# ameli/gaussian-process-param-estimation

Hardware: AMD Instinct MI355X
Metric: log-likelihood evals/sec (N=16384 dense Matern-3/2) (higher is better)
Workload: dtype f64

## Files before the change

### gaussian-process-param-estimation_amd/csrc/gpmi_api.hip

```cpp

#include <hip/hip_runtime.h>

#include <algorithm>
#include <cmath>
#include <cstdarg>
#include <cstdio>
#include <cstdlib>
#include <cstring>
#include <array>
#include <map>
#include <vector>

#include "gpmi_internal.h"
#include "gpmi_host.h"
#include "gpmi_band.h"
#include "../../include/gpmi.h"

using namespace gpmi;

namespace {

thread_local char g_err[512] = "";

int set_err(int code, const char* fmt, ...) {
  va_list ap;
  va_start(ap, fmt);
  vsnprintf(g_err, sizeof(g_err), fmt, ap);
  va_end(ap);
  return code;
}

constexpr int TS = GPMI_TS;
constexpr int RLD = GPMI_RHS_LD;
constexpr int OUT_LD = 1 + RLD * RLD;

}

struct gpmi_op {
  int device = 0;
  int64_t n = 0, n_pad = 0;
  int nt = 0;
  int max_batch = 1;
  int outer = 16;
  hipStream_t stream = nullptr;
  hipStream_t stream3 = nullptr;
  int groups = 0;
  hipEvent_t ev_g = nullptr;
  hipEvent_t ev_fork = nullptr, ev_join = nullptr;
  bool dry = false;
  std::vector<std::pair<int, int>> shapes;
  double* K = nullptr;
  double* A = nullptr;
  double* R = nullptr;
  double* X = nullptr;
  double* U = nullptr;
  double* Linv = nullptr;
  double* logdiag = nullptr;
  double* gram = nullptr;
  double* out = nullptr;
  double* etas = nullptr;
  double* rhs_src = nullptr;
  double* scratch = nullptr;
  double* scratch2 = nullptr;
  double* tracebuf = nullptr;
  double* W = nullptr;
  double* tpart = nullptr;
  double* Td = nullptr;
  int* info = nullptr;
  uint32_t* order = nullptr;
  int order_nt = -1, order_outer = -1, group = 8;
  std::map<std::pair<int, int>, int64_t> order_off;
  int nrhs = 0;
  bool has_K = false;
  bool cache_valid = false;
  double cached_eta = 0.0;
  uint64_t factor_gen = 0;
  uint64_t tinv_gen = ~0ull;
  int tinv_have = 0;
  double tinv[2] = {0.0, 0.0};
  bool timing = false;
  std::vector<hipEvent_t> ev;
  hipEvent_t ev_begin = nullptr, ev_end = nullptr;
  double last_syrk_ms = 0.0, last_syrk_flops = 0.0, last_total_ms = 0.0;
  int last_syrk_launches = 0;
  std::vector<std::pair<int, double>> syrk_log;
  std::vector<std::array<int, 3>> syrk_shape;
  double last_syrk_busy_ms = 0.0;

  BatchPtrs ptrs() const {
    BatchPtrs p;
    p.A = A;
    p.sA = n_pad * n_pad;
    p.R = R;
    p.sR = n_pad * RLD;
    p.U = U;
    p.sU = (int64_t)TS * RLD;
    p.Linv = Linv;
    p.sL = (int64_t)nt * TS * TS;
    p.logdiag = logdiag;
    p.sLD = nt;
    p.gram = gram;
    p.sG = (int64_t)nt * 256;
    p.info = info;
    return p;
  }
};

namespace {

void grouped_order(int w, int t, int G, std::vector<uint32_t>* out) {
  for (int r0 = 0; r0 < t; r0 += G) {
    const int r1 = std::min(t, r0 + G);
    const int jmax = std::min(r1 - 1, w - 1);
    for (int j = 0; j <= jmax; ++j)
      for (int i = std::max(r0, j); i < r1; ++i) out->push_back(((uint32_t)i << 16) | j);
  }
}

int launch_syrk(gpmi_op* op, hipStream_t st, int b0, int nb, int tc0, int w, int t, int p0,
                int kdim, bool from_k = false) {
  const int tri = w * (w + 1) / 2;
  const int tiles = tri + (t - w) * w;
  if (tiles <= 0 || nb <= 0) return 0;
  if (op->dry) {
    op->shapes.push_back({w, t});
    return 0;
  }
  int evi = -1;
  if (op->timing) {
    evi = (int)op->syrk_log.size() * 2;
    if ((int)op->ev.size() < evi + 2) {
      for (int k = 0; k < 64; ++k) {
        hipEvent_t e;
        HIP_TRY(hipEventCreateWithFlags(&e, timing_event_flags()));
        op->ev.push_back(e);
      }
    }
    HIP_TRY(hipEventRecord(op->ev[evi], st));
  }
  const uint32_t* order = nullptr;
  if (op->order && w > 1) {
    auto it = op->order_off.find({w, t});
    if (it != op->order_off.end()) order = op->order + it->second;
  }
  hipLaunchKernelGGL(syrk_kernel, dim3(tiles, nb), dim3(256), 0, st,
                     op->A + (int64_t)b0 * op->n_pad * op->n_pad, (int64_t)op->n_pad,
                     op->n_pad * op->n_pad, tc0, w, t, p0, kdim, order,
                     from_k ? op->K : nullptr, op->etas + b0, (int64_t)op->n);
  LAUNCH_CHECK("syrk_kernel");
  if (op->timing) {
    HIP_TRY(hipEventRecord(op->ev[evi + 1], st));
    const double offd = (double)(tiles - std::min(tiles, w)) * TS * TS;
    const double diag = (double)std::min(tiles, w) * TS * (TS + 1) / 2.0;
    const double fl = 2.0 * (offd + diag) * kdim * nb;
    op->syrk_log.push_back({evi, fl});
    op->syrk_shape.push_back({w, t, kdim});
  }
  return 0;
}

int factor_panel(gpmi_op* op, const BatchPtrs& P, int b0, int nb, hipStream_t st, int c0,
                 int W) {
  const int nt = op->nt;
  if (W == 1) {
    if (op->dry) return 0;
    hipLaunchKernelGGL(diag_block_kernel, dim3(nb), dim3(256), 0, st, P, (int64_t)op->n_pad,
                       c0, nt);
    LAUNCH_CHECK("diag_block_kernel");
    if (c0 + 1 < nt) {
      hipLaunchKernelGGL(panel_kernel, dim3(nt - c0 - 1, nb), dim3(256), 0, st, P,
                         (int64_t)op->n_pad, c0);
      LAUNCH_CHECK("panel_kernel");
    }
    return 0;
  }
  const int h = W / 2;
  int rc = factor_panel(op, P, b0, nb, st, c0, h);
  if (rc) return rc;
  rc = launch_syrk(op, st, b0, nb, c0 + h, W - h, nt - c0 - h, c0 * TS, h * TS);
  if (rc) return rc;
  return factor_panel(op, P, b0, nb, st, c0 + h, W - h);
}


int schedule(gpmi_op* op, const BatchPtrs& P, int b0, int nb, hipStream_t main = nullptr) {
  const int nt = op->nt, O = op->outer;
  hipStream_t A = main ? main : op->stream;
  for (int c0 = 0; c0 < nt; c0 += O) {
    const int W = std::min(O, nt - c0);
    int rc = factor_panel(op, P, b0, nb, A, c0, W);
    if (rc) return rc;
    const int c1 = c0 + W;
    if (c1 >= nt) break;
    rc = launch_syrk(op, A, b0, nb, c1, nt - c1, nt - c1, c0 * TS, W * TS, c0 == 0);
    if (rc) return rc;
  }
  return 0;
}

int ensure_order(gpmi_op* op) {
  if (op->group <= 0) return 0;
  if (op->order && op->order_nt == op->nt && op->order_outer == op->outer &&
      true)
    return 0;
  if (op->order) HIP_TRY(hipFree(op->order));
  op->order = nullptr;
  op->order_off.clear();
  op->dry = true;
  op->shapes.clear();
  BatchPtrs P = op->ptrs();
  int rc = schedule(op, P, 0, 1);
  op->dry = false;
  if (rc) return rc;
  std::vector<uint32_t> h;
  for (auto& wt : op->shapes) {
    if (wt.first < 2 || op->order_off.count(wt)) continue;
    op->order_off[wt] = (int64_t)h.size();
    grouped_order(wt.first, wt.second, op->group, &h);
  }
  if (h.empty()) h.push_back(0);
  HIP_TRY(hipMalloc(&op->order, sizeof(uint32_t) * h.size()));
  HIP_TRY(hipMemcpy(op->order, h.data(), sizeof(uint32_t) * h.size(), hipMemcpyHostToDevice));
  op->order_nt = op->nt;
  op->order_outer = op->outer;
  return 0;
}

BatchPtrs shifted(const BatchPtrs& P, int b0) {
  BatchPtrs q = P;
  q.A += b0 * P.sA;
  q.R += b0 * P.sR;
  q.U += b0 * P.sU;
  q.Linv += b0 * P.sL;
  q.logdiag += b0 * P.sLD;
  q.gram += b0 * P.sG;
  q.info += b0;
  return q;
}

int run_factor(gpmi_op* op, const double* etas_host, int nb, const double* rhs_dev) {
  if (!op->has_K) return set_err(-1000, "operator has no matrix (load or assemble first)");
  if (nb < 1 || nb > op->max_batch)
    return set_err(-1001, "batch %d outside [1, %d]", nb, op->max_batch);
  DeviceGuard g(op->device);
  hipStream_t s = op->stream;
  const int nt = op->nt;
  const int64_t lda = op->n_pad;
  BatchPtrs P = op->ptrs();
  {
    int rc = ensure_order(op);
    if (rc) return rc;
  }
  op->syrk_log.clear();
  op->syrk_shape.clear();
  op->cache_valid = false;
  ++op->factor_gen;
  if (op->timing) {
    if (!op->ev_begin) {
      HIP_TRY(hipEventCreateWithFlags(&op->ev_begin, timing_event_flags()));
      HIP_TRY(hipEventCreateWithFlags(&op->ev_end, timing_event_flags()));
    }
    HIP_TRY(hipEventRecord(op->ev_begin, s));
  }
  HIP_TRY(hipMemcpyAsync(op->etas, etas_host, sizeof(double) * nb, hipMemcpyHostToDevice, s));
  const int wc = std::min(op->outer, nt);
  hipLaunchKernelGGL(shift_copy_kernel, dim3(wc * (wc + 1) / 2 + (nt - wc) * wc), dim3(256), 0,
                     s, op->K, lda, op->A, lda, P.sA, op->etas, nb, op->n, wc);
  LAUNCH_CHECK("shift_copy_kernel");
  for (int b = 0; b < nb; ++b)
    HIP_TRY(hipMemcpyAsync(op->R + b * P.sR, rhs_dev, sizeof(double) * P.sR,
                           hipMemcpyDeviceToDevice, s));
  HIP_TRY(hipMemsetAsync(op->info, 0, sizeof(int) * nb, s));
  int rc = 0;
  const int groups = op->groups ? op->groups : (nb <= 32 ? 2 : 1);
  if (groups == 2 && nb >= 2) {
    const int h = nb / 2;
    if (!op->stream3) {
      HIP_TRY(hipStreamCreateWithFlags(&op->stream3, hipStreamNonBlocking));
      HIP_TRY(hipEventCreateWithFlags(&op->ev_g, sync_event_flags()));
    }
    HIP_TRY(hipEventRecord(op->ev_fork, s));
    HIP_TRY(hipStreamWaitEvent(op->stream3, op->ev_fork, 0));
    if ((rc = schedule(op, P, 0, h, s))) return rc;
    if ((rc = schedule(op, shifted(P, h), h, nb - h, op->stream3))) return rc;
    HIP_TRY(hipEventRecord(op->ev_g, op->stream3));
    HIP_TRY(hipStreamWaitEvent(s, op->ev_g, 0));
  } else {
    rc = schedule(op, P, 0, nb);
  }
  if (rc) return rc;
  hipLaunchKernelGGL(finalize_kernel, dim3(nb), dim3(256), 0, s, P, nt, op->out, OUT_LD);
  LAUNCH_CHECK("finalize_kernel");
  if (op->timing) HIP_TRY(hipEventRecord(op->ev_end, s));
  return 0;
}

int collect_timing(gpmi_op* op) {
  if (!op->timing) return 0;
  HIP_TRY(hipEventSynchronize(op->ev_end));
  double tot = 0.0, fl = 0.0;
  std::vector<std::pair<double, double>> iv;
  for (auto& pr : op->syrk_log) {
    float ms = 0.f, t0 = 0.f, t1 = 0.f;
    HIP_TRY(hipEventElapsedTime(&ms, op->ev[pr.first], op->ev[pr.first + 1]));
    HIP_TRY(hipEventElapsedTime(&t0, op->ev_begin, op->ev[pr.first]));
    HIP_TRY(hipEventElapsedTime(&t1, op->ev_begin, op->ev[pr.first + 1]));
    iv.push_back({t0, t1});
    tot += ms;
    fl += pr.second;
  }
  if (std::getenv("GPMI_SYRK_TRACE")) {
    std::map<std::pair<int, int>, std::array<double, 3>> cls;
    for (size_t i = 0; i < op->syrk_log.size(); ++i) {
      const auto& sh = op->syrk_shape[i];
      float ms = 0.f;
      HIP_TRY(hipEventElapsedTime(&ms, op->ev[op->syrk_log[i].first],
                                  op->ev[op->syrk_log[i].first + 1]));
      auto& c = cls[{sh[0] == sh[1] ? 1 : 0, sh[2]}];
      c[0] += 1;
      c[1] += ms;
      c[2] += op->syrk_log[i].second;
    }
    for (auto& kv : cls)
      fprintf(stderr, "[gpmi syrk] %s kdim=%4d launches=%3.0f ms=%8.3f TF/s=%6.2f\n",
              kv.first.first ? "bulk" : "band", kv.first.second, kv.second[0], kv.second[1],
              kv.second[2] / (kv.second[1] * 1e-3) / 1e12);
  }
  std::sort(iv.begin(), iv.end());
  double busy = 0.0, cs = -1.0, ce = -1.0;
  for (auto& x : iv) {
    if (x.first > ce) {
      if (ce > cs) busy += ce - cs;
      cs = x.first;
      ce = x.second;
    } else if (x.second > ce) {
      ce = x.second;
    }
  }
  if (ce > cs) busy += ce - cs;
  float all = 0.f;
  HIP_TRY(hipEventElapsedTime(&all, op->ev_begin, op->ev_end));
  op->last_syrk_ms = tot;
  op->last_syrk_busy_ms = busy;
  op->last_syrk_flops = fl;
  op->last_syrk_launches = (int)op->syrk_log.size();
  op->last_total_ms = all;
  return 0;
}

int upload_rhs(gpmi_op* op, double* dst, const double* rhs, int64_t ld, int nrhs, int col0) {
  std::vector<double> h((size_t)op->n_pad * RLD, 0.0);
  for (int64_t i = 0; i < op->n; ++i)
    for (int c = 0; c < nrhs; ++c) h[(size_t)i * RLD + c] = rhs[i * ld + col0 + c];
  HIP_TRY(hipMemcpyAsync(dst, h.data(), sizeof(double) * h.size(),
                         hipMemcpyHostToDevice, op->stream));
  HIP_TRY(hipStreamSynchronize(op->stream));
  return 0;
}

int ensure_factor(gpmi_op* op, double eta, const double* rhs_dev, bool* fresh) {
  *fresh = false;
  if (op->cache_valid && op->cached_eta == eta) return 0;
  int rc = run_factor(op, &eta, 1, rhs_dev);
  if (rc) return rc;
  op->cache_valid = true;
  op->cached_eta = eta;
  *fresh = true;
  return 0;
}

}

namespace gpmi {
int matern_params_host(double nu, MaternParams* P);
int set_error(int code, const char* msg) { return set_err(code, "%s", msg); }
int op_view(const gpmi_op* op, OpView* v) {
  if (!op) return set_err(-1006, "null handle");
  v->device = op->device;
  v->n = op->n;
  v->n_pad = op->n_pad;
  v->K = op->K;
  v->has_K = op->has_K;
  return 0;
}
}

namespace {
__global__ void pad_identity_kernel(double* K, int64_t ldk, int64_t n) {
  const int64_t i = n + threadIdx.x;
  if (i < ldk) K[i * ldk + i] = 1.0;
}
}

extern "C" {

int gpmi_version(void) { return 100; }

int gpmi_last_error(char* buf, size_t len) {
  if (!buf || !len) return 0;
  strncpy(buf, g_err, len - 1);
  buf[len - 1] = 0;
  return 0;
}

int gpmi_device_count(int* count) {
  HIP_TRY(hipGetDeviceCount(count));
  return 0;
}

// ... 21 lines not shown
}

int gpmi_matern_values(int device, const double* x, int64_t m, double nu, double* out) {
  if (m <= 0) return 0;
  MaternParams P;
  int rc = matern_params(nu, &P);
  if (rc) return rc;
  DeviceGuard g(device);
  double *dx = nullptr, *dv = nullptr;
  HIP_TRY(hipMalloc(&dx, sizeof(double) * m));
  HIP_TRY(hipMalloc(&dv, sizeof(double) * m));
  HIP_TRY(hipMemcpy(dx, x, sizeof(double) * m, hipMemcpyHostToDevice));
  hipLaunchKernelGGL(matern_eval_kernel, dim3((unsigned)((m + 255) / 256)), dim3(256), 0, 0, dx,
                     m, P, dv);
  LAUNCH_CHECK("matern_eval_kernel");
  HIP_TRY(hipMemcpy(out, dv, sizeof(double) * m, hipMemcpyDeviceToHost));
  HIP_TRY(hipFree(dx));
  HIP_TRY(hipFree(dv));
  return 0;
}

static int assemble(int device, hipStream_t s, const double* points, int64_t n, int d,
                    const double* scale, double nu, double* Kdev, int64_t ldk,
                    int64_t n_pad) {
  if (d < 1 || d > GPMI_MAX_DIM)
    return set_err(-1003, "dimension %d outside [1, %d]", d, GPMI_MAX_DIM);
  MaternParams P;
  int rc = matern_params(nu, &P);
  if (rc) return rc;
  DeviceGuard g(device);
  double *dp = nullptr, *ds = nullptr;
  HIP_TRY(hipMalloc(&dp, sizeof(double) * std::max<int64_t>(1, n * d)));
  HIP_TRY(hipMalloc(&ds, sizeof(double) * d));
  HIP_TRY(hipMemcpyAsync(dp, points, sizeof(double) * n * d, hipMemcpyHostToDevice, s));
  HIP_TRY(hipMemcpyAsync(ds, scale, sizeof(double) * d, hipMemcpyHostToDevice, s));
  const int64_t T = (n_pad + 63) / 64;
  hipEvent_t e0 = nullptr, e1 = nullptr;
  HIP_TRY(hipEventCreate(&e0));
  HIP_TRY(hipEventCreate(&e1));
  HIP_TRY(hipEventRecord(e0, s));
  launch_matern_dense(dim3((unsigned)(T * (T + 1) / 2)), s, dp, n, d, ds, P, Kdev, ldk, n_pad);
  LAUNCH_CHECK("matern_dense_kernel");
  HIP_TRY(hipEventRecord(e1, s));
  HIP_TRY(hipStreamSynchronize(s));
  float ms = 0.f;
  HIP_TRY(hipEventElapsedTime(&ms, e0, e1));
  g_assembly_ms = ms;
  HIP_TRY(hipEventDestroy(e0));
  HIP_TRY(hipEventDestroy(e1));
  HIP_TRY(hipFree(dp));
  HIP_TRY(hipFree(ds));
  return 0;
}

int gpmi_matern_dense(int device, const double* points, int64_t n, int d,
                      const double* scale, double nu, double* K_out, int64_t ldk) {
  if (n <= 0) return 0;
  DeviceGuard g(device);
  double* dK = nullptr;
  HIP_TRY(hipMalloc(&dK, sizeof(double) * n * n));
  int rc = assemble(device, nullptr, points, n, d, scale, nu, dK, n, n);
  if (rc) {
    (void)hipFree(dK);
    return rc;
  }
  HIP_TRY(hipMemcpy2D(K_out, sizeof(double) * ldk, dK, sizeof(double) * n, sizeof(double) * n,
                      n, hipMemcpyDeviceToHost));
  HIP_TRY(hipFree(dK));
  return 0;
}

int gpmi_op_create(int device, int64_t n, int max_batch, gpmi_op** out) {
  if (!out) return set_err(-1004, "null output handle");
  if (n <= 0) return set_err(-1005, "matrix size must be positive");
  if (max_batch < 1) max_batch = 1;
  DeviceGuard g(device);
  gpmi_op* op = new gpmi_op();
  op->device = device;
  op->n = n;
  op->n_pad = (n + TS - 1) / TS * TS;
  op->nt = (int)(op->n_pad / TS);
  op->max_batch = max_batch;
  if (const char* g = std::getenv("GPMI_GROUPS")) op->groups = std::atoi(g);
  const int64_t np = op->n_pad;
  auto fail = [&](hipError_t e, const char* what) {
    gpmi_op_destroy(op);
    return set_err(-(int)e, "allocation of %s failed: %s", what, hipGetErrorString(e));
  };
  hipError_t e;
  if ((e = hipStreamCreateWithFlags(&op->stream, hipStreamNonBlocking)) != hipSuccess)
    return fail(e, "stream");
  if ((e = hipEventCreateWithFlags(&op->ev_fork, sync_event_flags())) != hipSuccess)
    return fail(e, "event");
  if ((e = hipEventCreateWithFlags(&op->ev_join, sync_event_flags())) != hipSuccess)
    return fail(e, "event");
#define ALLOC(ptr, count)                                                           \
  if ((e = hipMalloc(&op->ptr, sizeof(*op->ptr) * (size_t)(count))) != hipSuccess)  \
    return fail(e, #ptr);
  ALLOC(K, np * np);
  ALLOC(A, (size_t)max_batch * np * np);
  ALLOC(R, (size_t)max_batch * np * RLD);
  ALLOC(X, (size_t)max_batch * np * RLD);
  ALLOC(U, (size_t)max_batch * TS * RLD);
  ALLOC(Linv, (size_t)max_batch * op->nt * TS * TS);
  ALLOC(logdiag, (size_t)max_batch * op->nt);
  ALLOC(gram, (size_t)max_batch * op->nt * 256);
  ALLOC(out, (size_t)max_batch * OUT_LD);
  ALLOC(etas, max_batch);
  ALLOC(rhs_src, np * RLD);
  ALLOC(scratch, np * RLD);
  ALLOC(scratch2, np * RLD);
  ALLOC(tracebuf, np * 2);
  ALLOC(info, max_batch);
#undef ALLOC
  if ((e = hipMemsetAsync(op->rhs_src, 0, sizeof(double) * np * RLD, op->stream)) != hipSuccess)
    return fail(e, "rhs memset");
  if ((e = hipStreamSynchronize(op->stream)) != hipSuccess) return fail(e, "sync");
  *out = op;
  return 0;
}

int gpmi_op_destroy(gpmi_op* op) {
  if (!op) return 0;
  DeviceGuard g(op->device);
  if (op->stream) (void)hipStreamSynchronize(op->stream);
  if (op->stream3) (void)hipStreamSynchronize(op->stream3);
  double* bufs[] = {op->K, op->A, op->R, op->X, op->U, op->Linv, op->logdiag, op->gram,
                    op->out, op->etas, op->rhs_src, op->scratch, op->scratch2, op->tracebuf,
                    op->W, op->tpart, op->Td};
  for (double* p : bufs)
    if (p) (void)hipFree(p);
  if (op->info) (void)hipFree(op->info);
  if (op->order) (void)hipFree(op->order);
  for (auto e : op->ev) (void)hipEventDestroy(e);
  if (op->ev_begin) (void)hipEventDestroy(op->ev_begin);
  if (op->ev_end) (void)hipEventDestroy(op->ev_end);
  if (op->ev_fork) (void)hipEventDestroy(op->ev_fork);
  if (op->ev_join) (void)hipEventDestroy(op->ev_join);
  if (op->stream3) (void)hipStreamDestroy(op->stream3);
  if (op->ev_g) (void)hipEventDestroy(op->ev_g);
  if (op->stream) (void)hipStreamDestroy(op->stream);
  delete op;
  return 0;
}

int gpmi_op_size(const gpmi_op* op, int64_t* n, int64_t* n_pad) {
  if (!op) return set_err(-1006, "null handle");
  if (n) *n = op->n;
  if (n_pad) *n_pad = op->n_pad;
  return 0;
}

int gpmi_op_load_matrix(gpmi_op* op, const double* K_host, int64_t ldk) {
  if (!op) return set_err(-1006, "null handle");
  DeviceGuard g(op->device);
  const int64_t np = op->n_pad, n = op->n;
  std::vector<double> pad_rows;
  HIP_TRY(hipMemsetAsync(op->K, 0, sizeof(double) * np * np, op->stream));
  HIP_TRY(hipMemcpy2DAsync(op->K, sizeof(double) * np, K_host, sizeof(double) * ldk,
                           sizeof(double) * n, n, hipMemcpyHostToDevice, op->stream));
  if (np > n) {
    std::vector<double> one(1, 1.0);
    for (int64_t i = n; i < np; ++i)
      HIP_TRY(hipMemcpyAsync(op->K + i * np + i, one.data(), sizeof(double),
                             hipMemcpyHostToDevice, op->stream));
  }
  HIP_TRY(hipStreamSynchronize(op->stream));
  op->has_K = true;
  op->cache_valid = false;
  return 0;
}

int gpmi_op_load_sparse(gpmi_op* op, const gpmi_sp* sp) {
  if (!op || !sp) return set_err(-1006, "null handle");
  int64_t n_sp = 0;
  if (int rc = gpmi_sp_info(sp, &n_sp, nullptr)) return rc;
  if (n_sp != op->n) return set_err(-1005, "sparse operator has n = %lld, dense has %lld",
                                    (long long)n_sp, (long long)op->n);
  DeviceGuard g(op->device);
  const int64_t np = op->n_pad;
  HIP_TRY(hipMemsetAsync(op->K, 0, sizeof(double) * np * np, op->stream));
  if (int rc = gpmi::sp_scatter_dense(sp, op->device, op->K, np, op->stream)) return rc;
  if (np > op->n) {
    hipLaunchKernelGGL(pad_identity_kernel, dim3(1), dim3(128), 0, op->stream, op->K, np, op->n);
    HIP_TRY(hipGetLastError());
  }
  HIP_TRY(hipStreamSynchronize(op->stream));
  op->has_K = true;
  op->cache_valid = false;
  return 0;
}

int gpmi_op_assemble_matern(gpmi_op* op, const double* points, int d, const double* scale,
                            double nu) {
  if (!op) return set_err(-1006, "null handle");
  int rc = assemble(op->device, op->stream, points, op->n, d, scale, nu, op->K, op->n_pad,
                    op->n_pad);
  if (rc) return rc;
  op->has_K = true;
  op->cache_valid = false;
  return 0;
}

int gpmi_op_get_matrix(gpmi_op* op, double* K_out, int64_t ldk) {
  if (!op) return set_err(-1006, "null handle");
  DeviceGuard g(op->device);
  HIP_TRY(hipMemcpy2DAsync(K_out, sizeof(double) * ldk, op->K, sizeof(double) * op->n_pad,
                           sizeof(double) * op->n, op->n, hipMemcpyDeviceToHost, op->stream));
  HIP_TRY(hipStreamSynchronize(op->stream));
  return 0;
}

int gpmi_op_set_rhs(gpmi_op* op, const double* rhs, int64_t ld, int nrhs) {
  if (!op) return set_err(-1006, "null handle");
  if (nrhs < 0 || nrhs > RLD) return set_err(-1007, "nrhs %d outside [0, %d]", nrhs, RLD);
  DeviceGuard g(op->device);
  int rc = upload_rhs(op, op->rhs_src, rhs, ld, nrhs, 0);
// ... 268 lines not shown
```

### gaussian-process-param-estimation_amd/csrc/gpmi_chol.hip

```cpp

#include <hip/hip_runtime.h>
#include <math.h>
#include <stdint.h>

#include "gpmi_internal.h"

#include "gpmi_device.h"

namespace gpmi {

__global__ __launch_bounds__(256) void shift_copy_kernel(
    const double* __restrict__ K, int64_t ldk, double* __restrict__ A, int64_t lda,
    int64_t sA, const double* __restrict__ etas, int nb, int64_t n, int wc) {
  int I, J;
  tri_decode(blockIdx.x, wc, &I, &J);
  const int t = threadIdx.x;
  for (int e = t; e < TS * TS / 2; e += 256) {
    const int r = e >> 6, c = (e & 63) * 2;
    const int64_t gi = (int64_t)I * TS + r, gj = (int64_t)J * TS + c;
    const d2 v = *reinterpret_cast<const d2*>(K + gi * ldk + gj);
    for (int b = 0; b < nb; ++b) {
      d2 o = v;
      if (gi < n) {
        if (gi == gj) o[0] += etas[b];
        if (gi == gj + 1) o[1] += etas[b];
      }
      *reinterpret_cast<d2*>(A + b * sA + gi * lda + gj) = o;
    }
  }
}

#ifndef GPMI_PROBE_PANEL_NO_RHS
#define GPMI_PROBE_PANEL_NO_RHS 0
#endif
__global__ __launch_bounds__(256, 2) void panel_kernel(BatchPtrs P, int64_t lda, int kb) {
  __shared__ double smem[4 * STAGE + TS * RLD];
  double* sA = smem;
  double* sB = smem + 2 * STAGE;
  double* sU = smem + 4 * STAGE;
  const int t = threadIdx.x, lane = t & 63, w = t >> 6;
  const int wr = w >> 1, wc = w & 1, fr = lane & 15, fk = lane >> 4;
  const int b = blockIdx.y;
  const int I = kb + 1 + blockIdx.x;
  double* A = P.A + b * P.sA;
  const double* U = P.U + b * P.sU;
  if (!GPMI_PROBE_PANEL_NO_RHS) {
    d2 v[4];
#pragma unroll
    for (int it = 0; it < 4; ++it)
      v[it] = *reinterpret_cast<const d2*>(U + 2 * (it * 256 + t));
#pragma unroll
    for (int it = 0; it < 4; ++it) *reinterpret_cast<d2*>(&sU[2 * (it * 256 + t)]) = v[it];
  }
  double* Aik = A + (int64_t)I * TS * lda + (int64_t)kb * TS;
  const double* Li = P.Linv + b * P.sL + (int64_t)kb * TS * TS;
  d4 acc[4][4];
  d4 racc[2];
#pragma unroll
  for (int i = 0; i < 4; ++i)
#pragma unroll
    for (int j = 0; j < 4; ++j) acc[i][j] = d4{0.0, 0.0, 0.0, 0.0};
  racc[0] = racc[1] = d4{0.0, 0.0, 0.0, 0.0};
#if GPMI_PROBE_PANEL_NO_RHS
  tile_mma<false>(Aik, lda, Li, TS, TS, sA, sB, acc, sU, racc);
#else
  tile_mma<true>(Aik, lda, Li, TS, TS, sA, sB, acc, sU, racc);
#endif
#pragma unroll
  for (int i = 0; i < 4; ++i)
#pragma unroll
    for (int j = 0; j < 4; ++j)
#pragma unroll
      for (int r = 0; r < 4; ++r)
        Aik[(int64_t)(wr * 64 + i * 16 + fk + 4 * r) * lda + wc * 64 + j * 16 + fr] =
            acc[i][j][r];
  double* R = P.R + b * P.sR + (int64_t)I * TS * RLD;
#if GPMI_PROBE_PANEL_NO_RHS
  return;
#endif
#pragma unroll
  for (int h = 0; h < 2; ++h)
#pragma unroll
    for (int r = 0; r < 4; ++r)
      R[(wr * 64 + wc * 32 + h * 16 + fk + 4 * r) * RLD + fr] -= racc[h][r];
}

__global__ __launch_bounds__(256, 2) void syrk_kernel(double* A, int64_t lda, int64_t sA,
                                                      int tc0, int w, int t, int p0,
                                                      int kdim, const uint32_t* order,
                                                      const double* __restrict__ Ksrc,
                                                      const double* __restrict__ etas,
                                                      int64_t n) {
  __shared__ double smem[4 * STAGE];
  const int tid = threadIdx.x, lane = tid & 63, wv = tid >> 6;
  const int wr = wv >> 1, wc = wv & 1, fr = lane & 15, fk = lane >> 4;
  const int q = xcd_remap(blockIdx.x, gridDim.x);
  int i, j;
  if (order) {
    const uint32_t o = order[q];
    i = (int)(o >> 16);
    j = (int)(o & 0xffffu);
  } else {
    tri_decode(q, w, &i, &j);
  }
  (void)t;
  const int I = tc0 + i, J = tc0 + j;
  double* Ab = A + blockIdx.y * sA;
  const double* P1 = Ab + (int64_t)I * TS * lda + p0;
  const double* P2 = Ab + (int64_t)J * TS * lda + p0;
  double* C = Ab + (int64_t)I * TS * lda + (int64_t)J * TS;
  const double* Cin = Ksrc ? Ksrc + (int64_t)I * TS * lda + (int64_t)J * TS : C;
  d4 acc[4][4];
#pragma unroll
  for (int a = 0; a < 4; ++a)
#pragma unroll
    for (int c = 0; c < 4; ++c)
#pragma unroll
      for (int r = 0; r < 4; ++r)
        acc[a][c][r] = Cin[(int64_t)(wr * 64 + a * 16 + fk + 4 * r) * lda + wc * 64 + c * 16 + fr];
  if (Ksrc && I == J && wr == wc) {
    const double eta = etas[blockIdx.y];
#pragma unroll
    for (int a = 0; a < 4; ++a)
#pragma unroll
      for (int r = 0; r < 4; ++r)
        if (fk + 4 * r == fr && (int64_t)I * TS + wr * 64 + a * 16 + fr < n) acc[a][a][r] += eta;
  }
  d4 dummy[2];
  tile_mma<false, true>(P1, lda, P2, lda, kdim, smem, smem + 2 * STAGE, acc, nullptr, dummy);
#pragma unroll
  for (int a = 0; a < 4; ++a)
#pragma unroll
    for (int c = 0; c < 4; ++c)
#pragma unroll
      for (int r = 0; r < 4; ++r)
        C[(int64_t)(wr * 64 + a * 16 + fk + 4 * r) * lda + wc * 64 + c * 16 + fr] = acc[a][c][r];
}

__global__ __launch_bounds__(256) void finalize_kernel(BatchPtrs P, int nt, double* out,
                                                       int out_ld) {
  const int b = blockIdx.x, t = threadIdx.x;
  double g = 0.0;
  for (int k = 0; k < nt; ++k) g += P.gram[b * P.sG + (int64_t)k * 256 + t];
  out[b * out_ld + 1 + t] = g;
  if (t == 0) {
    double s = 0.0;
    for (int k = 0; k < nt; ++k) s += P.logdiag[b * P.sLD + k];
    out[b * out_ld] = s;
  }
}

__global__ __launch_bounds__(256) void bwd_step_kernel(BatchPtrs P, int64_t lda, int kb,
                                                       double* X, int64_t sX) {
  __shared__ double Ys[TS * RLD];
  __shared__ double Xs[TS * RLD];
  const int t = threadIdx.x, b = blockIdx.y, jblk = blockIdx.x;
  const int row = t & 127, half = t >> 7;
  double* R = P.R + b * P.sR;
  const double* A = P.A + b * P.sA;
  const double* Li = P.Linv + b * P.sL + (int64_t)kb * TS * TS;
  for (int e = t; e < TS * RLD; e += 256) Ys[e] = R[(int64_t)kb * TS * RLD + e];
  __syncthreads();
  {
    double xv[8];
#pragma unroll
    for (int q = 0; q < 8; ++q) xv[q] = 0.0;
    for (int r = row; r < TS; ++r) {
      const double l = Li[r * TS + row];
#pragma unroll
      for (int q = 0; q < 8; ++q) xv[q] += l * Ys[r * RLD + half * 8 + q];
    }
#pragma unroll
    for (int q = 0; q < 8; ++q) Xs[row * RLD + half * 8 + q] = xv[q];
  }
  __syncthreads();
  if (jblk == 0) {
    double* Xb = X + b * sX + (int64_t)kb * TS * RLD;
    for (int e = t; e < TS * RLD; e += 256) Xb[e] = Xs[e];
  }
  if (kb == 0) return;
  const double* Lkj = A + (int64_t)kb * TS * lda + (int64_t)jblk * TS;
  const int c = row;
  double yv[8];
#pragma unroll
  for (int q = 0; q < 8; ++q) yv[q] = 0.0;
  for (int r = 0; r < TS; ++r) {
    const double l = Lkj[(int64_t)r * lda + c];
#pragma unroll
    for (int q = 0; q < 8; ++q) yv[q] += l * Xs[r * RLD + half * 8 + q];
  }
  double* Yj = R + (int64_t)jblk * TS * RLD;
#pragma unroll
  for (int q = 0; q < 8; ++q) Yj[c * RLD + half * 8 + q] -= yv[q];
}

__global__ __launch_bounds__(256) void gemv_sym_kernel(const double* __restrict__ K,
                                                       int64_t ldk, int64_t n,
                                                       const double* __restrict__ x,
                                                       int64_t ldx, int ncol,
                                                       double* __restrict__ y, double eta,
                                                       int exponent) {
  (void)eta;
  (void)exponent;
  const int lane = threadIdx.x & 63;
  const int64_t row = (int64_t)blockIdx.x * 4 + (threadIdx.x >> 6);
  if (row >= n) return;
  for (int c = 0; c < ncol; ++c) {
    double s = 0.0;
    for (int64_t j = lane; j < n; j += 64) s += K[row * ldk + j] * x[j * ldx + c];
#pragma unroll
    for (int off = 32; off > 0; off >>= 1) s += __shfl_xor(s, off);
    if (lane == 0) y[row * ldx + c] = s;
  }
}

__global__ __launch_bounds__(256) void trace_kernel(const double* __restrict__ K, int64_t ldk,
                                                    int64_t n, double* __restrict__ out) {
  __shared__ double s0[256], s1[256];
  const int t = threadIdx.x;
// ... 73 lines not shown
```

### gaussian-process-param-estimation_amd/csrc/gpmi_device.h

```cpp
#pragma once

#include <hip/hip_runtime.h>
#include <stdint.h>

#include "gpmi_internal.h"

namespace gpmi {

typedef double d4 __attribute__((ext_vector_type(4)));
typedef double d2 __attribute__((ext_vector_type(2)));

constexpr int TS = GPMI_TS;
constexpr int BK = 16;
constexpr int STAGE = TS * BK;

__device__ __forceinline__ int slab_off(int row, int k) {
  return row * BK + 2 * ((k >> 1) ^ ((row >> 1) & 7)) + (k & 1);
}
constexpr int RLD = GPMI_RHS_LD;

__device__ __forceinline__ void st_sc1(double* p, double v) {
  __hip_atomic_store(reinterpret_cast<unsigned long long*>(p),
                     (unsigned long long)__double_as_longlong(v), __ATOMIC_RELAXED,
                     __HIP_MEMORY_SCOPE_AGENT);
// ... 8 lines not shown
  return __builtin_amdgcn_mfma_f64_16x16x4f64(a, b, c, 0, 0, 0);
}

__device__ __forceinline__ d4 mfma64_neg(double a, double b, d4 c) {
  return __builtin_amdgcn_mfma_f64_16x16x4f64(a, b, c, 0, 0, 1);
}


__device__ __forceinline__ void gload_slab(const double* __restrict__ base, int64_t ld,
                                           int p, d2 (&r)[4]) {
  const int t = threadIdx.x;
#pragma unroll
  for (int i = 0; i < 4; ++i) {
    const int idx = i * 256 + t;
    const int row = idx >> 3, c2 = idx & 7;
    r[i] = *reinterpret_cast<const d2*>(base + (int64_t)row * ld + p + 2 * c2);
  }
}

__device__ __forceinline__ void sstore_slab(double* s, const d2 (&r)[4]) {
  const int t = threadIdx.x;
#pragma unroll
  for (int i = 0; i < 4; ++i) {
    const int idx = i * 256 + t;
    const int row = idx >> 3, c2 = idx & 7;
    *reinterpret_cast<d2*>(s + row * BK + 2 * (c2 ^ ((row >> 1) & 7))) = r[i];
  }
}


template <bool WITH_RHS, bool NEG = false>
__device__ __forceinline__ void tile_mma(const double* __restrict__ P1, int64_t ld1,
                                         const double* __restrict__ P2, int64_t ld2,
                                         int kdim, double* sA, double* sB,
                                         d4 (&acc)[4][4], const double* sU,
                                         d4 (&racc)[2]) {
  const int t = threadIdx.x, lane = t & 63, w = t >> 6;
  const int wr = w >> 1, wc = w & 1;
  const int fr = lane & 15, fk = lane >> 4;
  d2 ra[4], rb[4];
  gload_slab(P1, ld1, 0, ra);
  gload_slab(P2, ld2, 0, rb);
  sstore_slab(sA, ra);
  sstore_slab(sB, rb);
  __syncthreads();
  __builtin_amdgcn_s_waitcnt(0x0F70);
  const int nsteps = kdim / BK;
  for (int s = 0; s < nsteps; ++s) {
    const int cur = s & 1;
    const double* cA = sA + cur * STAGE;
    const double* cB = sB + cur * STAGE;
    if (s + 1 < nsteps) {
      gload_slab(P1, ld1, (s + 1) * BK, ra);
      gload_slab(P2, ld2, (s + 1) * BK, rb);
    }
#pragma unroll
    for (int kk = 0; kk < BK / 4; ++kk) {
      double a[4], b[4];
#pragma unroll
      for (int i = 0; i < 4; ++i) a[i] = cA[slab_off(wr * 64 + i * 16 + fr, kk * 4 + fk)];
#pragma unroll
      for (int j = 0; j < 4; ++j) b[j] = cB[slab_off(wc * 64 + j * 16 + fr, kk * 4 + fk)];
#pragma unroll
      for (int i = 0; i < 4; ++i)
#pragma unroll
        for (int j = 0; j < 4; ++j)
          acc[i][j] = NEG ? mfma64_neg(a[i], b[j], acc[i][j]) : mfma64(a[i], b[j], acc[i][j]);
      if (WITH_RHS) {
        const double u = sU[(s * BK + kk * 4 + fk) * RLD + fr];
        const double a0 = wc ? a[2] : a[0];
        const double a1 = wc ? a[3] : a[1];
        racc[0] = mfma64(a0, u, racc[0]);
        racc[1] = mfma64(a1, u, racc[1]);
      }
    }
    if (s + 1 < nsteps) {
      sstore_slab(sA + (cur ^ 1) * STAGE, ra);
      sstore_slab(sB + (cur ^ 1) * STAGE, rb);
    }
    __syncthreads();
  }
}

__device__ __forceinline__ int xcd_remap(int bid, int nwg) {
  const int xcd = bid & 7, q = nwg >> 3, r = nwg & 7;
  return (xcd < r ? xcd * (q + 1) : r * (q + 1) + (xcd - r) * q) + (bid >> 3);
}

__device__ __forceinline__ void tri_decode(int q, int w, int* pi, int* pj) {
  const int tri = w * (w + 1) / 2;
  int i, j;
  if (q < tri) {
    i = (int)((sqrt(8.0 * (double)q + 1.0) - 1.0) * 0.5);
    while ((i + 1) * (i + 2) / 2 <= q) ++i;
    while (i * (i + 1) / 2 > q) --i;
    j = q - i * (i + 1) / 2;
  } else {
    const int r = q - tri;
    i = w + r / w;
    j = r % w;
  }
  *pi = i;
  *pj = j;
}

}
```

### gaussian-process-param-estimation_amd/csrc/gpmi_internal.h

```cpp
#pragma once

#include <hip/hip_runtime.h>
#include <stdint.h>
#include <stdlib.h>

#include "gpmi_ms_sched.h"

#define GPMI_MAX_DIM 8
#define GPMI_TS 128
#define GPMI_RHS_LD 16

struct gpmi_sp;

namespace gpmi {

inline unsigned sync_event_flags() {
  static const unsigned f = [] {
    const char* e = getenv("GPMI_EV_SYSFENCE");
    return (unsigned)hipEventDisableTiming |
           ((e && e[0] == '1') ? 0u : (unsigned)hipEventDisableSystemFence);
  }();
  return f;
}
inline unsigned timing_event_flags() {
  return sync_event_flags() & ~(unsigned)hipEventDisableTiming;
}

enum MaternMode { MATERN_HALF = 0, MATERN_3HALF = 1, MATERN_5HALF = 2,
                  MATERN_GENERAL = 3, MATERN_GAUSS = 4 };

struct MaternParams {
  int mode;
  double nu;
  double sqrt2nu;
  double mu;
  double lp0, lp1;
};

void launch_matern_dense(dim3 grid, hipStream_t s, const double* points, int64_t n, int d,
                         const double* scale, const MaternParams& P, double* K, int64_t ldk,
                         int64_t n_pad);

struct BatchPtrs {
  double* A;        int64_t sA;
  double* R;        int64_t sR;
  double* U;        int64_t sU;
  double* Linv;     int64_t sL;
  double* logdiag;  int64_t sLD;
  double* gram;     int64_t sG;
  int* info;
};

__global__ void shift_copy_kernel(const double* K, int64_t ldk, double* A, int64_t lda,
                                  int64_t sA, const double* etas, int nb, int64_t n,
                                  int wc);
__global__ void diag_block_kernel(BatchPtrs P, int64_t lda, int kb, int nt);
__global__ void panel_kernel(BatchPtrs P, int64_t lda, int kb);
__global__ void syrk_kernel(double* A, int64_t lda, int64_t sA, int tc0, int w, int t,
                            int p0, int kdim, const uint32_t* order, const double* Ksrc,
                            const double* etas, int64_t n);
__global__ void finalize_kernel(BatchPtrs P, int nt, double* out, int out_ld);
__global__ void bwd_step_kernel(BatchPtrs P, int64_t lda, int kb, double* X, int64_t sX);
__global__ void fwd_step_kernel(BatchPtrs P, int64_t lda, int kb);
__global__ void gemv_sym_kernel(const double* K, int64_t ldk, int64_t n,
                                const double* x, int64_t ldx, int ncol, double* y,
                                double eta, int exponent);
__global__ void trace_kernel(const double* K, int64_t ldk, int64_t n, double* out);
__global__ void trinv_diag_kernel(const double* Linv, double* W, int64_t ldw, int k,
                                  double* partial);
__global__ void trinv_update_kernel(const double* L, int64_t lda, double* W, int64_t ldw, int i0,
                                    int nj, int kb, int ke);
__global__ void gram_panel_kernel(double* W, int64_t ldw, double* Td, int p0, int kdim,
                                  int imax);
__global__ void gram_sumsq_kernel(const double* W, int64_t ldw, const double* Td,
                                  double* partial);
__global__ void matern_eval_kernel(const double* x, int64_t m, MaternParams P, double* out);

#ifndef GPMI_LZ_JC
#define GPMI_LZ_JC 16
#endif
constexpr int LZ_JC = GPMI_LZ_JC;

struct MsScal {
  double* rr;
  double* a;
  double* a_prev;
  double* beta;
  int* active;
};
struct MsShift {
  double* bn2;
  double* z;
  double* z_prev;
  double* bp;
  double* g;
  int* flags;
  int* it_stop;
};
constexpr int MS_UB = 512;
constexpr int MS_DOT_BLK = 256;

constexpr int MS_CJOBS = 12;
struct MsCompactJob {
  const double* src;
  double* dst;
  int64_t rows;
  int L;
  int pad;
};
struct MsCompactArgs {
  MsCompactJob job[MS_CJOBS];
  int njob, s, a, nd, s0, pad;
  int map[MS_MAXS];
  int drop[MS_MAXS];
  int drop_orig[MS_MAXS];
  const double* g;
  double* gfin;
  int64_t SN;
  const int* act_src;
  int* act;
};

int sp_scatter_dense(const ::gpmi_sp* sp, int device, double* K, int64_t ldk,
                     hipStream_t st);

}
```

Baseline: 44.32.

## Add column-panel Cholesky schedule and triangular-aware panel TRSM

Moves the dense Cholesky launch sequence into a plan generator and adds an optional left-looking column-panel mode (GPMI_PANEL=col). In that mode a fused kernel applies the pending update to the panel, then does the triangular solve, and can update the next diagonal block. Separately, the default panel kernel now uses a tile_trsm routine that skips MFMA work on the zero half of the triangular inverse. This cuts panel FLOPs. The new column mode is off by default and gives up recursive SYRK parallelism in exchange for fewer launches.

After: 45.03 (median of 6 runs). 1.6% higher.

```diff
diff --git a/gaussian-process-param-estimation_amd/csrc/gpmi_api.hip b/gaussian-process-param-estimation_amd/csrc/gpmi_api.hip
--- a/gaussian-process-param-estimation_amd/csrc/gpmi_api.hip
+++ b/gaussian-process-param-estimation_amd/csrc/gpmi_api.hip
@@ -14,6 +14,7 @@
 #include "gpmi_internal.h"
 #include "gpmi_host.h"
 #include "gpmi_band.h"
+#include "gpmi_dense_plan.h"
 #include "../../include/gpmi.h"
 
 using namespace gpmi;
@@ -42,6 +43,7 @@
   int nt = 0;
   int max_batch = 1;
   int outer = 16;
+  int panel_mode = DENSE_REC;
   hipStream_t stream = nullptr;
   hipStream_t stream3 = nullptr;
   int groups = 0;
@@ -86,6 +88,9 @@
   std::vector<std::pair<int, double>> syrk_log;
   std::vector<std::array<int, 3>> syrk_shape;
   double last_syrk_busy_ms = 0.0;
+  bool trace = false;
+  std::vector<hipEvent_t> colpanel_ev;
+  size_t colpanel_ev_used = 0;
 
   BatchPtrs ptrs() const {
     BatchPtrs p;
@@ -159,40 +164,46 @@
   return 0;
 }
 
-int factor_panel(gpmi_op* op, const BatchPtrs& P, int b0, int nb, hipStream_t st, int c0,
-                 int W) {
-  const int nt = op->nt;
-  if (W == 1) {
-    if (op->dry) return 0;
-    hipLaunchKernelGGL(diag_block_kernel, dim3(nb), dim3(256), 0, st, P, (int64_t)op->n_pad,
-                       c0, nt);
+int factor_panel(gpmi_op* op, const BatchPtrs& P, int nb, hipStream_t st,
+                 const DenseLaunch& L) {
+  if (op->dry) return 0;
+  const int64_t lda = op->n_pad;
+  if (L.kind == DENSE_DIAG) {
+    hipLaunchKernelGGL(diag_block_kernel, dim3(nb), dim3(256), 0, st, P, lda, L.col, op->nt);
     LAUNCH_CHECK("diag_block_kernel");
-    if (c0 + 1 < nt) {
-      hipLaunchKernelGGL(panel_kernel, dim3(nt - c0 - 1, nb), dim3(256), 0, st, P,
-                         (int64_t)op->n_pad, c0);
-      LAUNCH_CHECK("panel_kernel");
-    }
-    return 0;
-  }
-  const int h = W / 2;
-  int rc = factor_panel(op, P, b0, nb, st, c0, h);
-  if (rc) return rc;
-  rc = launch_syrk(op, st, b0, nb, c0 + h, W - h, nt - c0 - h, c0 * TS, h * TS);
-  if (rc) return rc;
-  return factor_panel(op, P, b0, nb, st, c0 + h, W - h);
+  } else if (L.kind == DENSE_PANEL) {
+    hipLaunchKernelGGL(panel_kernel, dim3(L.r1 - L.r0, nb), dim3(256), 0, st, P, lda, L.col);
+    LAUNCH_CHECK("panel_kernel");
+  } else {
+    const bool ev = op->timing && op->trace;
+    size_t evi = op->colpanel_ev_used;
+    if (ev) {
+      while (op->colpanel_ev.size() < evi + 2) {
+        hipEvent_t e;
+        HIP_TRY(hipEventCreateWithFlags(&e, timing_event_flags()));
+        op->colpanel_ev.push_back(e);
+      }
+      HIP_TRY(hipEventRecord(op->colpanel_ev[evi], st));
+    }
+    hipLaunchKernelGGL(colpanel_kernel, dim3(L.r1 - L.r0, nb), dim3(256), 0, st, P, lda, L.col,
+                       L.p0 / TS, L.next_diag ? 1 : 0);
+    LAUNCH_CHECK("colpanel_kernel");
+    if (ev) {
+      HIP_TRY(hipEventRecord(op->colpanel_ev[evi + 1], st));
+      op->colpanel_ev_used = evi + 2;
+    }
+  }
+  return 0;
 }
 
 
 int schedule(gpmi_op* op, const BatchPtrs& P, int b0, int nb, hipStream_t main = nullptr) {
-  const int nt = op->nt, O = op->outer;
   hipStream_t A = main ? main : op->stream;
-  for (int c0 = 0; c0 < nt; c0 += O) {
-    const int W = std::min(O, nt - c0);
-    int rc = factor_panel(op, P, b0, nb, A, c0, W);
-    if (rc) return rc;
-    const int c1 = c0 + W;
-    if (c1 >= nt) break;
-    rc = launch_syrk(op, A, b0, nb, c1, nt - c1, nt - c1, c0 * TS, W * TS, c0 == 0);
+  for (const DenseLaunch& L : dense_plan(op->nt, op->outer, op->panel_mode)) {
+    const int rc = L.kind == DENSE_SYRK
+                       ? launch_syrk(op, A, b0, nb, L.col, L.w, L.r1 - L.r0, L.p0, L.kdim,
+                                     L.from_k)
+                       : factor_panel(op, P, nb, A, L);
     if (rc) return rc;
   }
   return 0;
@@ -253,6 +264,7 @@
   }
   op->syrk_log.clear();
   op->syrk_shape.clear();
+  op->colpanel_ev_used = 0;
   op->cache_valid = false;
   ++op->factor_gen;
   if (op->timing) {
@@ -309,7 +321,7 @@
     tot += ms;
     fl += pr.second;
   }
-  if (std::getenv("GPMI_SYRK_TRACE")) {
+  if (op->trace) {
     std::map<std::pair<int, int>, std::array<double, 3>> cls;
     for (size_t i = 0; i < op->syrk_log.size(); ++i) {
       const auto& sh = op->syrk_shape[i];
@@ -325,6 +337,15 @@
       fprintf(stderr, "[gpmi syrk] %s kdim=%4d launches=%3.0f ms=%8.3f TF/s=%6.2f\n",
               kv.first.first ? "bulk" : "band", kv.first.second, kv.second[0], kv.second[1],
               kv.second[2] / (kv.second[1] * 1e-3) / 1e12);
+    double cp = 0.0;
+    for (size_t i = 0; i + 1 < op->colpanel_ev_used; i += 2) {
+      float ms = 0.f;
+      HIP_TRY(hipEventElapsedTime(&ms, op->colpanel_ev[i], op->colpanel_ev[i + 1]));
+      cp += ms;
+    }
+    if (op->colpanel_ev_used)
+      fprintf(stderr, "[gpmi syrk] colpanel_kernel launches=%3zu ms=%8.3f\n",
+              op->colpanel_ev_used / 2, cp);
   }
   std::sort(iv.begin(), iv.end());
   double busy = 0.0, cs = -1.0, ce = -1.0;
@@ -512,6 +533,14 @@
   op->nt = (int)(op->n_pad / TS);
   op->max_batch = max_batch;
   if (const char* g = std::getenv("GPMI_GROUPS")) op->groups = std::atoi(g);
+  if (const char* m = std::getenv("GPMI_PANEL")) {
+    if (!std::strcmp(m, "col")) op->panel_mode = DENSE_COL;
+    else if (std::strcmp(m, "rec") && *m) {
+      delete op;
+      return set_err(-1011, "GPMI_PANEL must be rec or col (got %s)", m);
+    }
+  }
+  op->trace = std::getenv("GPMI_SYRK_TRACE") != nullptr;
   const int64_t np = op->n_pad;
   auto fail = [&](hipError_t e, const char* what) {
     gpmi_op_destroy(op);
@@ -563,6 +592,7 @@
   if (op->info) (void)hipFree(op->info);
   if (op->order) (void)hipFree(op->order);
   for (auto e : op->ev) (void)hipEventDestroy(e);
+  for (auto e : op->colpanel_ev) (void)hipEventDestroy(e);
   if (op->ev_begin) (void)hipEventDestroy(op->ev_begin);
   if (op->ev_end) (void)hipEventDestroy(op->ev_end);
   if (op->ev_fork) (void)hipEventDestroy(op->ev_fork);
diff --git a/gaussian-process-param-estimation_amd/csrc/gpmi_chol.hip b/gaussian-process-param-estimation_amd/csrc/gpmi_chol.hip
--- a/gaussian-process-param-estimation_amd/csrc/gpmi_chol.hip
+++ b/gaussian-process-param-estimation_amd/csrc/gpmi_chol.hip
@@ -33,56 +33,125 @@
 #ifndef GPMI_PROBE_PANEL_NO_RHS
 #define GPMI_PROBE_PANEL_NO_RHS 0
 #endif
+__device__ __forceinline__ void panel_step(double* Aik, int64_t lda, const double* Li,
+                                           double* R, double* sA, double* sB,
+                                           const double* sU) {
+  const int t = threadIdx.x, lane = t & 63, w = t >> 6;
+  const int wr = w >> 1, wc = w & 1, fr = lane & 15, fk = lane >> 4;
+  d4 acc[4][4];
+  d4 racc[2];
+#pragma unroll
+  for (int i = 0; i < 4; ++i)
+#pragma unroll
+    for (int j = 0; j < 4; ++j) acc[i][j] = d4{0.0, 0.0, 0.0, 0.0};
+  racc[0] = racc[1] = d4{0.0, 0.0, 0.0, 0.0};
+#if GPMI_PROBE_PANEL_NO_RHS
+  tile_trsm<false>(Aik, lda, Li, sA, sB, acc, sU, racc);
+#else
+  tile_trsm<true>(Aik, lda, Li, sA, sB, acc, sU, racc);
+#endif
+#pragma unroll
+  for (int i = 0; i < 4; ++i)
+#pragma unroll
+    for (int j = 0; j < 4; ++j)
+#pragma unroll
+      for (int r = 0; r < 4; ++r)
+        Aik[(int64_t)(wr * 64 + i * 16 + fk + 4 * r) * lda + trsm_cb(wc, j) * 16 + fr] =
+            acc[i][j][r];
+#if GPMI_PROBE_PANEL_NO_RHS
+  return;
+#endif
+#pragma unroll
+  for (int h = 0; h < 2; ++h)
+#pragma unroll
+    for (int r = 0; r < 4; ++r)
+      R[(wr * 64 + wc * 32 + h * 16 + fk + 4 * r) * RLD + fr] -= racc[h][r];
+}
+
+__device__ __forceinline__ void stage_u(const double* U, double* sU) {
+  const int t = threadIdx.x;
+  d2 v[4];
+#pragma unroll
+  for (int it = 0; it < 4; ++it) v[it] = *reinterpret_cast<const d2*>(U + 2 * (it * 256 + t));
+#pragma unroll
+  for (int it = 0; it < 4; ++it) *reinterpret_cast<d2*>(&sU[2 * (it * 256 + t)]) = v[it];
+}
+
+__device__ __forceinline__ void wg_global_barrier() {
+  __builtin_amdgcn_fence(__ATOMIC_RELEASE, "workgroup");
+  __syncthreads();
+  __builtin_amdgcn_fence(__ATOMIC_ACQUIRE, "workgroup");
+}
+
 __global__ __launch_bounds__(256, 2) void panel_kernel(BatchPtrs P, int64_t lda, int kb) {
+  __shared__ double smem[4 * STAGE + TS * RLD];
+  double* sU = smem + 4 * STAGE;
+  const int b = blockIdx.y;
+  const int I = kb + 1 + blockIdx.x;
+  double* A = P.A + b * P.sA;
+  if (!GPMI_PROBE_PANEL_NO_RHS) stage_u(P.U + b * P.sU, sU);
+  panel_step(A + (int64_t)I * TS * lda + (int64_t)kb * TS, lda,
+             P.Linv + b * P.sL + (int64_t)kb * TS * TS,
+             P.R + b * P.sR + (int64_t)I * TS * RLD, smem, smem + 2 * STAGE, sU);
+}
+
+__device__ __forceinline__ void load_c(const double* C, int64_t lda, d4 (&acc)[4][4]) {
+  const int tid = threadIdx.x, lane = tid & 63, wv = tid >> 6;
+  const int wr = wv >> 1, wc = wv & 1, fr = lane & 15, fk = lane >> 4;
+#pragma unroll
+  for (int a = 0; a < 4; ++a)
+#pragma unroll
+    for (int c = 0; c < 4; ++c)
+#pragma unroll
+      for (int r = 0; r < 4; ++r)
+        acc[a][c][r] = C[(int64_t)(wr * 64 + a * 16 + fk + 4 * r) * lda + wc * 64 + c * 16 + fr];
+}
+__device__ __forceinline__ void store_c(double* C, int64_t lda, const d4 (&acc)[4][4]) {
+  const int tid = threadIdx.x, lane = tid & 63, wv = tid >> 6;
+  const int wr = wv >> 1, wc = wv & 1, fr = lane & 15, fk = lane >> 4;
+#pragma unroll
+  for (int a = 0; a < 4; ++a)
+#pragma unroll
+    for (int c = 0; c < 4; ++c)
+#pragma unroll
+      for (int r = 0; r < 4; ++r)
+        C[(int64_t)(wr * 64 + a * 16 + fk + 4 * r) * lda + wc * 64 + c * 16 + fr] = acc[a][c][r];
+}
+
+__global__ __launch_bounds__(256, 2) void colpanel_kernel(BatchPtrs P, int64_t lda, int kb,
+                                                          int c0, int next_diag) {
   __shared__ double smem[4 * STAGE + TS * RLD];
   double* sA = smem;
   double* sB = smem + 2 * STAGE;
   double* sU = smem + 4 * STAGE;
-  const int t = threadIdx.x, lane = t & 63, w = t >> 6;
-  const int wr = w >> 1, wc = w & 1, fr = lane & 15, fk = lane >> 4;
   const int b = blockIdx.y;
   const int I = kb + 1 + blockIdx.x;
+  const int kdim = (kb - c0) * TS;
   double* A = P.A + b * P.sA;
-  const double* U = P.U + b * P.sU;
-  if (!GPMI_PROBE_PANEL_NO_RHS) {
-    d2 v[4];
-#pragma unroll
-    for (int it = 0; it < 4; ++it)
-      v[it] = *reinterpret_cast<const d2*>(U + 2 * (it * 256 + t));
-#pragma unroll
-    for (int it = 0; it < 4; ++it) *reinterpret_cast<d2*>(&sU[2 * (it * 256 + t)]) = v[it];
-  }
-  double* Aik = A + (int64_t)I * TS * lda + (int64_t)kb * TS;
-  const double* Li = P.Linv + b * P.sL + (int64_t)kb * TS * TS;
-  d4 acc[4][4];
-  d4 racc[2];
-#pragma unroll
-  for (int i = 0; i < 4; ++i)
-#pragma unroll
-    for (int j = 0; j < 4; ++j) acc[i][j] = d4{0.0, 0.0, 0.0, 0.0};
-  racc[0] = racc[1] = d4{0.0, 0.0, 0.0, 0.0};
-#if GPMI_PROBE_PANEL_NO_RHS
-  tile_mma<false>(Aik, lda, Li, TS, TS, sA, sB, acc, sU, racc);
-#else
-  tile_mma<true>(Aik, lda, Li, TS, TS, sA, sB, acc, sU, racc);
-#endif
-#pragma unroll
-  for (int i = 0; i < 4; ++i)
-#pragma unroll
-    for (int j = 0; j < 4; ++j)
-#pragma unroll
-      for (int r = 0; r < 4; ++r)
-        Aik[(int64_t)(wr * 64 + i * 16 + fk + 4 * r) * lda + wc * 64 + j * 16 + fr] =
-            acc[i][j][r];
-  double* R = P.R + b * P.sR + (int64_t)I * TS * RLD;
-#if GPMI_PROBE_PANEL_NO_RHS
-  return;
-#endif
-#pragma unroll
-  for (int h = 0; h < 2; ++h)
-#pragma unroll
-    for (int r = 0; r < 4; ++r)
-      R[(wr * 64 + wc * 32 + h * 16 + fk + 4 * r) * RLD + fr] -= racc[h][r];
+  stage_u(P.U + b * P.sU, sU);
+  double* rowI = A + (int64_t)I * TS * lda;
+  double* Aik = rowI + (int64_t)kb * TS;
+  d4 dummy[2];
+  if (kdim > 0) {
+    d4 acc[4][4];
+    load_c(Aik, lda, acc);
+    tile_mma<false, true>(rowI + (int64_t)c0 * TS, lda,
+                          A + (int64_t)kb * TS * lda + (int64_t)c0 * TS, lda, kdim, sA, sB, acc,
+                          nullptr, dummy);
+    store_c(Aik, lda, acc);
+    wg_global_barrier();
+  }
+  panel_step(Aik, lda, P.Linv + b * P.sL + (int64_t)kb * TS * TS,
+             P.R + b * P.sR + (int64_t)I * TS * RLD, sA, sB, sU);
+  if (next_diag && blockIdx.x == 0) {
+    wg_global_barrier();
+    double* D = rowI + (int64_t)I * TS;
+    d4 acc[4][4];
+    load_c(D, lda, acc);
+    tile_mma<false, true>(rowI + (int64_t)c0 * TS, lda, rowI + (int64_t)c0 * TS, lda,
+                          kdim + TS, sA, sB, acc, nullptr, dummy);
+    store_c(D, lda, acc);
+  }
 }
 
 __global__ __launch_bounds__(256, 2) void syrk_kernel(double* A, int64_t lda, int64_t sA,
@@ -111,13 +180,7 @@
   double* C = Ab + (int64_t)I * TS * lda + (int64_t)J * TS;
   const double* Cin = Ksrc ? Ksrc + (int64_t)I * TS * lda + (int64_t)J * TS : C;
   d4 acc[4][4];
-#pragma unroll
-  for (int a = 0; a < 4; ++a)
-#pragma unroll
-    for (int c = 0; c < 4; ++c)
-#pragma unroll
-      for (int r = 0; r < 4; ++r)
-        acc[a][c][r] = Cin[(int64_t)(wr * 64 + a * 16 + fk + 4 * r) * lda + wc * 64 + c * 16 + fr];
+  load_c(Cin, lda, acc);
   if (Ksrc && I == J && wr == wc) {
     const double eta = etas[blockIdx.y];
 #pragma unroll
@@ -128,13 +191,7 @@
   }
   d4 dummy[2];
   tile_mma<false, true>(P1, lda, P2, lda, kdim, smem, smem + 2 * STAGE, acc, nullptr, dummy);
-#pragma unroll
-  for (int a = 0; a < 4; ++a)
-#pragma unroll
-    for (int c = 0; c < 4; ++c)
-#pragma unroll
-      for (int r = 0; r < 4; ++r)
-        C[(int64_t)(wr * 64 + a * 16 + fk + 4 * r) * lda + wc * 64 + c * 16 + fr] = acc[a][c][r];
+  store_c(C, lda, acc);
 }
 
 __global__ __launch_bounds__(256) void finalize_kernel(BatchPtrs P, int nt, double* out,
diff --git a/gaussian-process-param-estimation_amd/csrc/gpmi_dense_plan.h b/gaussian-process-param-estimation_amd/csrc/gpmi_dense_plan.h
--- /dev/null
+++ b/gaussian-process-param-estimation_amd/csrc/gpmi_dense_plan.h
@@ -0,0 +1,62 @@
+#pragma once
+
+#include <algorithm>
+#include <vector>
+
+#pragma GCC visibility push(hidden)
+
+namespace gpmi {
+
+constexpr int DENSE_TS = 128;
+
+enum DenseMode { DENSE_REC = 0, DENSE_COL = 1 };
+enum DenseKind { DENSE_DIAG = 0, DENSE_PANEL = 1, DENSE_COLPANEL = 2, DENSE_SYRK = 3 };
+
+struct DenseLaunch {
+  int kind;
+  int col;
+  int w;
+  int r0, r1;
+  int p0, kdim;
+  bool next_diag;
+  bool from_k;
+};
+
+inline void dense_plan_rec(int nt, int c0, int W, std::vector<DenseLaunch>* out) {
+  if (W == 1) {
+    out->push_back({DENSE_DIAG, c0, 1, c0, c0 + 1, 0, 0, false, false});
+    if (c0 + 1 < nt) out->push_back({DENSE_PANEL, c0, 1, c0 + 1, nt, 0, 0, false, false});
+    return;
+  }
+  const int h = W / 2;
+  dense_plan_rec(nt, c0, h, out);
+  out->push_back({DENSE_SYRK, c0 + h, W - h, c0 + h, nt, c0 * DENSE_TS, h * DENSE_TS, false,
+                  false});
+  dense_plan_rec(nt, c0 + h, W - h, out);
+}
+
+inline std::vector<DenseLaunch> dense_plan(int nt, int outer, int mode) {
+  std::vector<DenseLaunch> out;
+  for (int c0 = 0; c0 < nt; c0 += outer) {
+    const int W = std::min(outer, nt - c0);
+    if (mode == DENSE_REC) {
+      dense_plan_rec(nt, c0, W, &out);
+    } else {
+      for (int k = c0; k < c0 + W; ++k) {
+        out.push_back({DENSE_DIAG, k, 1, k, k + 1, 0, 0, false, false});
+        if (k + 1 < nt)
+          out.push_back({DENSE_COLPANEL, k, 1, k + 1, nt, c0 * DENSE_TS, (k - c0) * DENSE_TS,
+                         k + 1 < c0 + W, false});
+      }
+    }
+    const int c1 = c0 + W;
+    if (c1 >= nt) break;
+    out.push_back({DENSE_SYRK, c1, nt - c1, c1, nt, c0 * DENSE_TS, W * DENSE_TS, false,
+                   c0 == 0});
+  }
+  return out;
+}
+
+}
+
+#pragma GCC visibility pop
diff --git a/gaussian-process-param-estimation_amd/csrc/gpmi_device.h b/gaussian-process-param-estimation_amd/csrc/gpmi_device.h
--- a/gaussian-process-param-estimation_amd/csrc/gpmi_device.h
+++ b/gaussian-process-param-estimation_amd/csrc/gpmi_device.h
@@ -114,6 +114,61 @@
   }
 }
 
+__device__ __forceinline__ int trsm_cb(int wc, int j) { return 2 * j + ((j ^ wc) & 1); }
+
+template <bool WITH_RHS>
+__device__ __forceinline__ void tile_trsm(const double* P1, int64_t ld1, const double* Linv,
+                                          double* sA, double* sB, d4 (&acc)[4][4],
+                                          const double* sU, d4 (&racc)[2]) {
+  const int t = threadIdx.x, lane = t & 63;
+  const int w = __builtin_amdgcn_readfirstlane(t >> 6);
+  const int wr = w >> 1, wc = w & 1;
+  const int fr = lane & 15, fk = lane >> 4;
+  d2 ra[4], rb[4];
+  gload_slab(P1, ld1, 0, ra);
+  gload_slab(Linv, TS, 0, rb);
+  sstore_slab(sA, ra);
+  sstore_slab(sB, rb);
+  __syncthreads();
+  constexpr int nsteps = TS / BK;
+#pragma unroll
+  for (int s = 0; s < nsteps; ++s) {
+    const int cur = s & 1;
+    const double* cA = sA + cur * STAGE;
+    const double* cB = sB + cur * STAGE;
+    if (s + 1 < nsteps) {
+      gload_slab(P1, ld1, (s + 1) * BK, ra);
+      gload_slab(Linv, TS, (s + 1) * BK, rb);
+    }
+#pragma unroll
+    for (int kk = 0; kk < BK / 4; ++kk) {
+      double a[4];
+#pragma unroll
+      for (int i = 0; i < 4; ++i) a[i] = cA[slab_off(wr * 64 + i * 16 + fr, kk * 4 + fk)];
+#pragma unroll
+      for (int j = 0; j < 4; ++j) {
+        if (s <= 2 * j || (s == 2 * j + 1 && ((j ^ wc) & 1))) {
+          const double bj = cB[slab_off(trsm_cb(wc, j) * 16 + fr, kk * 4 + fk)];
+#pragma unroll
+          for (int i = 0; i < 4; ++i) acc[i][j] = mfma64(a[i], bj, acc[i][j]);
+        }
+      }
+      if (WITH_RHS) {
+        const double u = sU[(s * BK + kk * 4 + fk) * RLD + fr];
+        const double a0 = wc ? a[2] : a[0];
+        const double a1 = wc ? a[3] : a[1];
+        racc[0] = mfma64(a0, u, racc[0]);
+        racc[1] = mfma64(a1, u, racc[1]);
+      }
+    }
+    if (s + 1 < nsteps) {
+      sstore_slab(sA + (cur ^ 1) * STAGE, ra);
+      sstore_slab(sB + (cur ^ 1) * STAGE, rb);
+    }
+    __syncthreads();
+  }
+}
+
 __device__ __forceinline__ int xcd_remap(int bid, int nwg) {
   const int xcd = bid & 7, q = nwg >> 3, r = nwg & 7;
   return (xcd < r ? xcd * (q + 1) : r * (q + 1) + (xcd - r) * q) + (bid >> 3);
diff --git a/gaussian-process-param-estimation_amd/csrc/gpmi_internal.h b/gaussian-process-param-estimation_amd/csrc/gpmi_internal.h
--- a/gaussian-process-param-estimation_amd/csrc/gpmi_internal.h
+++ b/gaussian-process-param-estimation_amd/csrc/gpmi_internal.h
@@ -56,6 +56,7 @@
                                   int wc);
 __global__ void diag_block_kernel(BatchPtrs P, int64_t lda, int kb, int nt);
 __global__ void panel_kernel(BatchPtrs P, int64_t lda, int kb);
+__global__ void colpanel_kernel(BatchPtrs P, int64_t lda, int kb, int c0, int next_diag);
 __global__ void syrk_kernel(double* A, int64_t lda, int64_t sA, int tc0, int w, int t,
                             int p0, int kdim, const uint32_t* order, const double* Ksrc,
                             const double* etas, int64_t n);
```
